# aidagroup/quad-periodic-mpc

Measured on AMD Instinct MI355X. Metric: QP solves/sec (N=10, 13-state, 12-force) at batch=65536; 1/2/4/8 GPU, higher is better.
Workload: dtype f32

## Files before the change

### quad-periodic-mpc_amd/csrc/cmpc_class1.hip

```cpp
#include <stdlib.h>

#include "cmpc_common.h"

#ifndef CMPC_W1_WAVES_60
#define CMPC_W1_WAVES_60 4
#endif
#ifndef CMPC_W1_WAVES_PER_EU
#define CMPC_W1_WAVES_PER_EU 4
#endif
#ifndef CMPC_C1_RL
#define CMPC_C1_RL 0
#endif
#ifndef CMPC_TRIP_PRIO_AT
#define CMPC_TRIP_PRIO_AT 0
#endif
#ifndef CMPC_C1_TRIP_PRIO
#define CMPC_C1_TRIP_PRIO 2
#endif
#ifndef C1_PIPE_GRP
#define C1_PIPE_GRP 4
#endif
#ifndef CMPC_C1_CHOL2
#define CMPC_C1_CHOL2 1
#endif
// ... 54 lines not shown
  static constexpr int PSZ = 4 * NG * NV - 8 * NG * (NG - 1);
  __host__ __device__ static constexpr int prow(int r) {
    return 4 * (r >> 2) * NV - 8 * (r >> 2) * ((r >> 2) - 1) + (r & 3) * (NV - 4 * (r >> 2));
  }
  __host__ __device__ static constexpr int prow0(int r) { return prow(r) - (r & ~3); }
  __host__ __device__ static constexpr int tri(int r) { return r * NV - ((r * (r + 1)) >> 1); }
  static_assert(NV * NV - ((NV * (NV + 1)) >> 1) <= 4 * NG * NV - 8 * NG * (NG - 1), "exchange fits P");
};
__device__ __forceinline__ int rcol(int j) { return (j * (j + 1)) >> 1; }
constexpr int rinv_cols(int words) {
  int q = 0;
  while ((q + 1) * (q + 2) <= words) q++;
  return q;
}

constexpr int OFF_E = 0;
constexpr int OFF_ZE = OFF_E + 16 * MAXN;
constexpr int OFF_REC = OFF_ZE + 16 * MAXN;

constexpr int C1_MAXFS = 24;

template <int NV>
struct SharedC1 {
  static_assert(NV % 4 == 0 && NV <= NL, "row width");
  static_assert(NV * (NV + 1) / 2 <= C1Geo<NV>::PSZ, "R must fit in P");
  static_assert(OFF_REC + CMPC_REC_WORDS(MAXN) <= C1Geo<NV>::PSZ, "prep scratch must fit in P");
  static_assert(3 * C1_MAXFS >= NV, "stance list");
  static_assert(NV * (NV + 1) / 2 <= C1Geo<NV>::PSZ - NL, "vbuf in P's tail");
  __device__ __forceinline__ float* vbuf() { return &P[C1Geo<NV>::PSZ - NL]; }
  static constexpr int QI = rinv_cols(C1Geo<NV>::PSZ - NL);
  static constexpr int RB = C1Geo<NV>::PSZ - NL - QI * (QI + 1) / 2;
  static_assert(QI * (QI + 1) / 2 <= RB, "R and R^-1 side by side");
  float P[C1Geo<NV>::PSZ];
  union {
    float BdtT[12][16];
    float ibuf[NL];
    struct {
      float bufA[NL], bufB[NL];
      float cs[2 * NL];
    } gi;
  } u;
  float sub[C1_MAXFS];
  int sfs[C1_MAXFS];
  int blkbase[MAXN + 2];
  unsigned char varblk[NL], varcol[NL];
  unsigned char cmask[NL];
};

__device__ __forceinline__ void lsync() {
  __builtin_amdgcn_wave_barrier();
  asm volatile("" ::: "memory");
}

__device__ __forceinline__ float fdiv(float a, float b) { return a * fast_rcp(b); }

template <int M>
__device__ __forceinline__ void pin(float (&x)[M]) {
#pragma unroll
  for (int c = 0; c < M; c++) asm volatile("" : "+v"(x[c]));
}

template <int LO, int HI, int MA>
__device__ __forceinline__ float pick_col(const float (&x)[MA], int q) {
  static_assert(0 <= LO && LO < HI && HI <= MA, "column range");
  if constexpr (HI - LO == 1) {
    float r = x[LO];
    asm volatile("" : "+v"(r));
    return r;
  } else {
    constexpr int MID = (LO + HI) / 2;
    if (q < MID) return pick_col<LO, MID>(x, q);
    return pick_col<MID, HI>(x, q);
  }
}

#ifndef CMPC_FENCE_COLS
#define CMPC_FENCE_COLS 16
#endif
#define CMPC_SWEEP_FENCE(c)                                                                  \
  do {                                                                                       \
    if (((c) & (CMPC_FENCE_COLS - 1)) == CMPC_FENCE_COLS - 4) __builtin_amdgcn_sched_barrier(0); \
  } while (0)

template <int NV>
__device__ __forceinline__ void solve_c1(const float* __restrict__ rec, const KParams& P,
                                         SharedC1<NV>& sh, float* __restrict__ fout,
                                         uint8_t* __restrict__ st_out, int32_t* __restrict__ it_out,
                                         int* __restrict__ ovf_list, int* __restrict__ ovf_count,
                                         int inst) {
  using G = C1Geo<NV>;
  const int v = threadIdx.x;
  const int N = P.N;
#ifdef CMPC_PHASE_PROF
  unsigned long long ph[16] = {0, 0, 0, 0, 0, 0, 0, 0, 0, 0, 0, 0, 0, 0, 0, 0};
  unsigned long long t_sub = 0;
  unsigned long long t_last = clock64();
#endif
  {
    const float4* src = reinterpret_cast<const float4*>(rec);
    float4* dst = reinterpret_cast<float4*>(&sh.P[OFF_REC]);
    for (int t = v; t < (P.rec_words >> 2); t += 64) dst[t] = src[t];
  }
  lsync();
  const float* srec = &sh.P[OFF_REC];
  const unsigned char* gait = reinterpret_cast<const unsigned char*>(srec + CMPC_REC_HDR + 12 * N);
  int nfs = 0;
  unsigned long long msk0 = 0ull, msk1 = 0ull;
  for (int c0 = 0; c0 < 4 * N; c0 += 64) {
    const int t = c0 + v;
    float ub = 0.f;
    bool f = false;
    if (t < 4 * N) {
      ub = (float)gait[t] * P.f_max;
      f = !(ub < 0.01f && ub > -0.01f);
    }
    const unsigned long long m = __ballot(f);
    if (c0 == 0) msk0 = m; else msk1 = m;
    const int pre = __popcll(m & ((1ull << v) - 1ull));
    if (f && nfs + pre < C1_MAXFS) {
      sh.sfs[nfs + pre] = t;
      sh.sub[nfs + pre] = ub;
    }
    nfs += __popcll(m);
  }
  const int n = 3 * nfs;
  if (n > NV) {
    if (v == 0 && ovf_list) ovf_list[atomicAdd(ovf_count, 1)] = inst;
    return;
  }
  lsync();
  {
    int kb = 0, kc = 0;
    if (v < n) {
      const int fs = sh.sfs[v / 3];
      kb = fs >> 2;
      kc = 3 * (fs & 3) + v % 3;
    }
    sh.varblk[v] = (unsigned char)kb;
    sh.varcol[v] = (unsigned char)kc;
    if (v <= N) {
      const int b0 = 4 * v, b1 = 4 * v - 64;
      const unsigned long long lo = (b0 >= 64) ? msk0 : (msk0 & ((1ull << b0) - 1ull));
      const unsigned long long hi = (b1 <= 0) ? 0ull : (msk1 & ((1ull << b1) - 1ull));
      sh.blkbase[v] = 3 * (__popcll(lo) + __popcll(hi));
    }
    for (int t = v; t < nfs; t += 64) sh.cmask[t] = 0;
  }
  Model md;
  make_model(srec, P.dt, md);
  make_bdt<64>(srec, md, v, sh.u.BdtT);
  CondGeo cg;
  make_cond_geo<true>(srec, md, cg);
  lsync();
  if (v < N) {
    float e[13];
    state_error(srec, md, v, srec + CMPC_REC_HDR + 12 * v, e);
#pragma unroll
    for (int j = 0; j < 13; j++) sh.P[OFF_E + 16 * v + j] = e[j];
  }
  lsync();
  float wts[13];
#pragma unroll
  for (int j = 0; j < 12; j++) wts[j] = P.wts[j];
  wts[12] = 0.f;
  {
    float ze[13];
#pragma unroll
    for (int j = 0; j < 13; j++) ze[j] = 0.f;
    for (int i = N - 1; i >= 0; i--) {
      float e[13];
#pragma unroll
      for (int j = 0; j < 13; j++) e[j] = sh.P[OFF_E + 16 * i + j];
      recur(md, wts, e, ze);
      float mine = 0.f;
#pragma unroll
      for (int j = 0; j < 13; j++) mine = (v == j) ? ze[j] : mine;
      if (v < 13) sh.P[OFF_ZE + 16 * i + v] = mine;
    }
  }
  lsync();
  C1_MARK(0);

  const bool real = v < n;
  float gv;
  {
    const int kv = real ? sh.varblk[v] : 0;
    const int cv = real ? sh.varcol[v] : 0;
    float b[13], u1[13], u2[13];
#pragma unroll
    for (int j = 0; j < 13; j++) b[j] = real ? sh.u.BdtT[cv][j] : 0.f;
    n1_mul(md, b, u1);
    n1_mul(md, u1, u2);
    {
      float zk[13];
#pragma unroll
      for (int j = 0; j < 13; j++) zk[j] = sh.P[OFF_ZE + 16 * kv + j];
      gv = real ? 2.f * dot13(b, zk) : 0.f;
    }
    lsync();
    const int myrow = G::tri(v);
    float z[13];
#pragma unroll
    for (int j = 0; j < 13; j++) z[j] = 0.f;
    for (int i = N - 1; i >= 0; i--) {
      const bool act = real && (i >= kv);
      const float k = (float)(i - kv);
      const float k2 = 0.5f * k * (k - 1.f);
      float gk[13];
      col_power(b, u1, u2, k, k2, gk);
#pragma unroll
      for (int j = 0; j < 13; j++) gk[j] = act ? gk[j] : 0.f;
      recur(md, wts, gk, z);
      asm volatile("" ::: "memory");
      const int wb = __builtin_amdgcn_readfirstlane(sh.blkbase[i]);
      step_entries(md, cg, sh.u.BdtT, step_mask(msk0, msk1, i), wb, z, [&](int w, float val) {
        if (w == v) val += P.alpha2;
        if (act && w >= v) sh.P[myrow + w] = val;
      });
    }
  }
  lsync();
  C1_MARK(1);

  float slot[NV + 1];
  {
    const int vv = (v < NV) ? v : 0;
    const int myrow = G::tri(vv);
    static_for<0, NV>([&](auto C) {
      constexpr int c = decltype(C)::value;
      const int addr = (c >= vv) ? myrow + c : G::tri(c) + vv;
      const float x = sh.P[addr];
      slot[c] = (real && c < n) ? x : ((c == v) ? 1.f : 0.f);
      if ((c & 7) == 7) __builtin_amdgcn_sched_barrier(0);
    });
    slot[NV] = gv;
  }
  lsync();

  int status = CMPC_OK;
  float my_inv = 1.f;
#if CMPC_C1_CHOL2
  float i0n = 1.f, betan = 0.f, i1n = 1.f, g0n = 0.f, g1n = 0.f;
  auto look = [&](auto JJ) {
    constexpr int j = decltype(JJ)::value, j1 = j + 1;
    constexpr int cj = j & ~3, cj1 = j1 & ~3;
    if constexpr (j1 < NV) {
    float d0 = rl(slot[j], j);
    const float h10 = rl(slot[j], j1);
    if (!(d0 > 0.f)) { status = CMPC_NOT_PD; d0 = 1e-30f; }
    i0n = __builtin_amdgcn_rsqf(d0);
    betan = h10 * (i0n * i0n);
    float d1 = fmaf(-h10, betan, rl(slot[j1], j1));
    if (!(d1 > 0.f)) { status = CMPC_NOT_PD; d1 = 1e-30f; }
    i1n = __builtin_amdgcn_rsqf(d1);
    g0n = rl(slot[NV], j);
    g1n = fmaf(-betan, g0n, rl(slot[NV], j1));
    const float s1 = fmaf(-slot[j], betan, slot[j1]);
#if CMPC_C1_FUSEDJ
    g0n = -g0n * i0n;
    g1n = -g1n * i1n;
    if (v >= cj && v < NV) sh.P[G::prow(j) + v - cj] = (v >= j) ? -slot[j] * i0n : 0.f;
    if (v >= cj1 && v < NV) sh.P[G::prow(j1) + v - cj1] = (v >= j1) ? -s1 * i1n : 0.f;
#else
    if (v >= cj && v < NV) sh.P[G::prow(j) + v - cj] = (v >= j) ? slot[j] : 0.f;
    if (v >= cj1 && v < NV) sh.P[G::prow(j1) + v - cj1] = (v >= j1) ? s1 : 0.f;
#endif
    lsync();
    }
  };
  if (n > 0) look(std::integral_constant<int, 0>{});
  float jc2 = 0.f, jc3 = 0.f;
  (void)jc2; (void)jc3;
  float xunc = 0.f;
  (void)xunc;
  static_for<0, NV / 2>([&](auto KB) {
    constexpr int k = 2 * decltype(KB)::value;
    constexpr int k1 = k + 1, k2 = k + 2;
    constexpr int c0 = k & ~3, c1 = k1 & ~3, c2 = k2 & ~3;
    constexpr int rk = G::prow(k), rk1 = G::prow(k1);
    if (k < n) {
      const float i0 = i0n, beta = betan, i1 = i1n, g0 = g0n, g1 = g1n;
#if CMPC_C1_FUSEDJ
      if (v == k) my_inv = i0;
      if (v == k1) my_inv = i1;
      const float s0 = slot[k];
      const float s1 = fmaf(-s0, beta, slot[k1]);
      const float a0 = (v > k) ? s0 * i0 : 0.f;
      const float a1 = (v > k1) ? s1 * i1 : 0.f;
#else
      if (v == k) { my_inv = i0; sh.u.ibuf[k] = i0; }
      if (v == k1) { my_inv = i1; sh.u.ibuf[k1] = i1; }
      const float s0 = slot[k];
      const float s1 = fmaf(-s0, beta, slot[k1]);
      const float a0 = (v > k) ? -s0 * (i0 * i0) : 0.f;
      const float a1 = (v > k1) ? -s1 * (i1 * i1) : 0.f;
#endif
      slot[NV] = fmaf(a1, g1, fmaf(a0, g0, slot[NV]));
      static_for<c2 / 4, NV / 4>([&](auto JC) {
        constexpr int c = 4 * decltype(JC)::value;
        const float4 r0 = *reinterpret_cast<const float4*>(&sh.P[rk + c - c0]);
        const float4 r1 = *reinterpret_cast<const float4*>(&sh.P[rk1 + c - c1]);
        axpy4(a0, r0, slot[c + 0], slot[c + 1], slot[c + 2], slot[c + 3]);
        axpy4(a1, r1, slot[c + 0], slot[c + 1], slot[c + 2], slot[c + 3]);
        if constexpr (k2 < NV && c == c2) {
          if (k2 < n) look(std::integral_constant<int, k2>{});
        }
        CMPC_SWEEP_FENCE(c);
      });
#if CMPC_C1_FUSEDJ == 2
      if constexpr ((k & 3) == 0) {
        f2v t0 = {(v == k) ? 1.f : 0.f, 0.f}, t1 = {(v == k1) ? 1.f : 0.f, 0.f};
        f2v t2 = {(v == k + 2) ? 1.f : 0.f, 0.f}, t3 = {(v == k + 3) ? 1.f : 0.f, 0.f};
#if CMPC_C1_JPIPE
        piped_sweep<0, k, 1>(
            [&](auto C) {
              constexpr int q = decltype(C)::value;
              return F4x4{*reinterpret_cast<const float4*>(&sh.P[G::prow(q) + k - q]),
                          *reinterpret_cast<const float4*>(&sh.P[G::prow(q + 1) + k - q]),
                          *reinterpret_cast<const float4*>(&sh.P[G::prow(q + 2) + k - q]),
                          *reinterpret_cast<const float4*>(&sh.P[G::prow(q + 3) + k - q])};
            },
            [&](auto C, F4x4 l) {
              constexpr int q = decltype(C)::value;
              const float4 la = l.a, lb = l.b, lc = l.c, ld = l.d;
#else
        static_for<0, k / 4>([&](auto QC) {
          constexpr int q = 4 * decltype(QC)::value;
          const float4 la = *reinterpret_cast<const float4*>(&sh.P[G::prow(q) + k - q]);
          const float4 lb = *reinterpret_cast<const float4*>(&sh.P[G::prow(q + 1) + k - q]);
          const float4 lc = *reinterpret_cast<const float4*>(&sh.P[G::prow(q + 2) + k - q]);
          const float4 ld = *reinterpret_cast<const float4*>(&sh.P[G::prow(q + 3) + k - q]);
#endif
          t0.x = fmaf(slot[q], la.x, t0.x); t1.x = fmaf(slot[q], la.y, t1.x);
          t2.x = fmaf(slot[q], la.z, t2.x); t3.x = fmaf(slot[q], la.w, t3.x);
          t0.y = fmaf(slot[q + 1], lb.x, t0.y); t1.y = fmaf(slot[q + 1], lb.y, t1.y);
          t2.y = fmaf(slot[q + 1], lb.z, t2.y); t3.y = fmaf(slot[q + 1], lb.w, t3.y);
          t0.x = fmaf(slot[q + 2], lc.x, t0.x); t1.x = fmaf(slot[q + 2], lc.y, t1.x);
          t2.x = fmaf(slot[q + 2], lc.z, t2.x); t3.x = fmaf(slot[q + 2], lc.w, t3.x);
          t0.y = fmaf(slot[q + 3], ld.x, t0.y); t1.y = fmaf(slot[q + 3], ld.y, t1.y);
          t2.y = fmaf(slot[q + 3], ld.z, t2.y); t3.y = fmaf(slot[q + 3], ld.w, t3.y);
#if CMPC_C1_JPIPE
            });
#else
          __builtin_amdgcn_sched_barrier(0);
        });
#endif
        const float hk = sh.P[G::prow(k) + k1 - (k & ~3)];
        const float xk = (t0.x + t0.y) * i0;
        slot[k] = xk;
        slot[k1] = fmaf(xk, hk, t1.x + t1.y) * i1;
#if CMPC_C1_XUNC
// ... 502 lines not shown
```

### quad-periodic-mpc_amd/csrc/cmpc_common.h

```cpp
#pragma once
#include <hip/hip_runtime.h>
#include <stdint.h>

#include <type_traits>

#include "cmpc_kernels.h"

namespace cmpc {
namespace {

constexpr int MAXN = CMPC_MAX_HORIZON;
constexpr float kBigF = 3.0e38f;

__device__ __forceinline__ float rl(float x, int lane) {
  return __int_as_float(__builtin_amdgcn_readlane(__float_as_int(x), lane));
}
__device__ __forceinline__ int rli(int x, int lane) { return __builtin_amdgcn_readlane(x, lane); }

constexpr int kDppQuadSwap1 = 0xB1;
constexpr int kDppQuadSwap2 = 0x4E;
constexpr int kDppRowShl = 0x100;
constexpr int kDppRowShr = 0x110;
constexpr int kDppWaveShl1 = 0x130;
constexpr int kDppWaveShr1 = 0x138;
// ... 56 lines not shown
  const int row = lane >> 4;
  return v + ((row == 0) ? r1 + (r2 + r3) : (row == 1) ? r2 + r3 : (row == 2) ? r3 : 0.f);
}
__device__ __forceinline__ float lane_prev(float old, float v) { return dppf<kDppWaveShr1>(old, v); }
__device__ __forceinline__ float lane_next(float old, float v) { return dppf<kDppWaveShl1>(old, v); }
__device__ __forceinline__ int lane_next_i(int old, int v) { return dppi<kDppWaveShl1>(old, v); }

__device__ __forceinline__ int tid_opq() {
  int x = threadIdx.x;
  asm volatile("" : "+v"(x));
  return x;
}

#ifndef CMPC_LANE_ASM
#define CMPC_LANE_ASM 1
#endif
__device__ __forceinline__ int lane_opq() {
#if CMPC_LANE_ASM
  int x;
  asm volatile("v_mbcnt_lo_u32_b32 %0, -1, 0\n\tv_mbcnt_hi_u32_b32 %0, -1, %0" : "=v"(x));
#else
  int x = (int)__builtin_amdgcn_mbcnt_hi(~0u, __builtin_amdgcn_mbcnt_lo(~0u, 0u));
  asm volatile("" : "+v"(x));
#endif
  return x;
}

template <int I, int E, class F>
__device__ __forceinline__ void static_for(F&& f) {
  if constexpr (I < E) {
    f(std::integral_constant<int, I>{});
    static_for<I + 1, E>(f);
  }
}
template <int C0, int CE, int GRP, class Ld, class F>
__device__ __forceinline__ void piped_sweep(Ld&& ld, F&& f) {
  constexpr int NCH = (CE > C0) ? (CE - C0) / 4 : 0;
  if constexpr (NCH > 0) {
    using T = decltype(ld(std::integral_constant<int, C0>{}));
    constexpr int NG = (NCH + GRP - 1) / GRP;
    T cur[GRP], nxt[GRP];
    static_for<0, GRP>([&](auto I) {
      constexpr int ch = decltype(I)::value;
      if constexpr (ch < NCH) cur[ch] = ld(std::integral_constant<int, C0 + 4 * ch>{});
    });
    static_for<0, NG>([&](auto GI) {
      constexpr int g = decltype(GI)::value;
      static_for<0, GRP>([&](auto I) {
        constexpr int ch = (g + 1) * GRP + decltype(I)::value;
        if constexpr (ch < NCH) nxt[decltype(I)::value] = ld(std::integral_constant<int, C0 + 4 * ch>{});
      });
      __builtin_amdgcn_sched_barrier(0);
      static_for<0, GRP>([&](auto I) {
        constexpr int ch = g * GRP + decltype(I)::value;
        if constexpr (ch < NCH) f(std::integral_constant<int, C0 + 4 * ch>{}, cur[decltype(I)::value]);
      });
      __builtin_amdgcn_sched_barrier(0);
      static_for<0, GRP>([&](auto I) { cur[decltype(I)::value] = nxt[decltype(I)::value]; });
    });
  }
}
struct F4x2 {
  float4 a, b;
};
struct F4x4 {
  float4 a, b, c, d;
};

__device__ __forceinline__ float vopq(float x) {
  asm volatile("" : "+v"(x));
  return x;
}
__device__ __forceinline__ float sopq(float x) {
  asm volatile("" : "+s"(x));
  return x;
}
__device__ __forceinline__ float rfl(float x) {
  return __int_as_float(__builtin_amdgcn_readfirstlane(__float_as_int(x)));
}
__device__ __forceinline__ int opaque(int x) {
  x = __builtin_amdgcn_readfirstlane(x);
  asm volatile("" : "+s"(x));
  return x;
}
__device__ __forceinline__ float fast_rcp(float x) { return __builtin_amdgcn_rcpf(x); }

typedef float f2v __attribute__((ext_vector_type(2)));
__device__ __forceinline__ void axpy4(float a, float4 r, float& x0, float& x1, float& x2, float& x3) {
  x0 = fmaf(a, r.x, x0);
  x1 = fmaf(a, r.y, x1);
  x2 = fmaf(a, r.z, x2);
  x3 = fmaf(a, r.w, x3);
}
__device__ __forceinline__ void dot4(f2v& acc, float x0, float x1, float x2, float x3, float4 r) {
  acc.x = fmaf(x0, r.x, acc.x);
  acc.x = fmaf(x1, r.y, acc.x);
  acc.x = fmaf(x2, r.z, acc.x);
  acc.x = fmaf(x3, r.w, acc.x);
}
__device__ __forceinline__ void dot4x2(f2v& acc, float x0, float x1, float x2, float x3, float4 r) {
  acc.x = fmaf(x0, r.x, acc.x);
  acc.y = fmaf(x1, r.y, acc.y);
  acc.x = fmaf(x2, r.z, acc.x);
  acc.y = fmaf(x3, r.w, acc.y);
}

__device__ __forceinline__ void wsync() {
  __builtin_amdgcn_fence(__ATOMIC_RELEASE, "workgroup");
  __builtin_amdgcn_wave_barrier();
  __builtin_amdgcn_fence(__ATOMIC_ACQUIRE, "workgroup");
}

struct Model {
  float R[9];
  float n1r[9];
  float dt, dth, xdrag;
};

__device__ __forceinline__ void n1_mul(const Model& m, const float* x, float* y) {
#pragma unroll
  for (int i = 0; i < 3; i++) y[i] = m.n1r[i * 3 + 0] * x[6] + m.n1r[i * 3 + 1] * x[7] + m.n1r[i * 3 + 2] * x[8];
  y[3] = m.dt * x[9];
  y[4] = m.dt * x[10];
  y[5] = m.dt * x[11] + (m.dth * m.xdrag) * x[9] + m.dth * x[12];
#pragma unroll
  for (int i = 6; i < 11; i++) y[i] = 0.f;
  y[11] = (m.dt * m.xdrag) * x[9] + m.dt * x[12];
  y[12] = 0.f;
}

__device__ __forceinline__ void recur(const Model& m, const float* wts, const float* e, float* z) {
  float t[13];
#pragma unroll
  for (int j = 0; j < 13; j++) t[j] = z[j];
  const float c6 = m.n1r[0] * t[0] + m.n1r[3] * t[1] + m.n1r[6] * t[2];
  const float c7 = m.n1r[1] * t[0] + m.n1r[4] * t[1] + m.n1r[7] * t[2];
  const float c8 = m.n1r[2] * t[0] + m.n1r[5] * t[1] + m.n1r[8] * t[2];
  const float c9 = m.dt * t[3] + (m.dt * m.xdrag) * t[11] + (m.dth * m.xdrag) * t[5];
  const float c10 = m.dt * t[4];
  const float c11 = m.dt * t[5];
  const float c12 = m.dt * t[11] + m.dth * t[5];
#pragma unroll
  for (int j = 0; j < 13; j++) z[j] = wts[j] * e[j] + t[j];
  z[6] += c6; z[7] += c7; z[8] += c8; z[9] += c9; z[10] += c10; z[11] += c11; z[12] += c12;
}

__device__ __forceinline__ float dot13(const float* a, const float* b) {
  float s = 0.f;
#pragma unroll
  for (int j = 0; j < 13; j++) s = fmaf(a[j], b[j], s);
  return s;
}

__device__ __forceinline__ unsigned step_mask(unsigned long long m0, unsigned long long m1, int i) {
  return (unsigned)(((i < 16) ? (m0 >> (4 * i)) : (m1 >> (4 * i - 64))) & 15ull);
}

#ifndef CMPC_COND_DOT13
#define CMPC_COND_DOT13 0
#endif

struct CondGeo {
  float Ii[9];
  float r[12];
};
struct StepProj {
  float w[3], p[3];
};

__device__ __forceinline__ void make_iinv(const Model& md, float* Ii) {
  const float Ib0 = .07f, Ib1 = 0.26f, Ib2 = 0.242f;
  float Iw[9];
#pragma unroll
  for (int i = 0; i < 3; i++)
#pragma unroll
    for (int j = 0; j < 3; j++)
      Iw[i * 3 + j] = md.R[i * 3 + 0] * Ib0 * md.R[j * 3 + 0] + md.R[i * 3 + 1] * Ib1 * md.R[j * 3 + 1] +
                      md.R[i * 3 + 2] * Ib2 * md.R[j * 3 + 2];
  const float c00 = Iw[4] * Iw[8] - Iw[5] * Iw[7];
  const float c10 = Iw[5] * Iw[6] - Iw[3] * Iw[8];
  const float c20 = Iw[3] * Iw[7] - Iw[4] * Iw[6];
  const float idet = 1.f / (Iw[0] * c00 + Iw[1] * c10 + Iw[2] * c20);
  Ii[0] = c00 * idet; Ii[1] = (Iw[2] * Iw[7] - Iw[1] * Iw[8]) * idet; Ii[2] = (Iw[1] * Iw[5] - Iw[2] * Iw[4]) * idet;
  Ii[3] = c10 * idet; Ii[4] = (Iw[0] * Iw[8] - Iw[2] * Iw[6]) * idet; Ii[5] = (Iw[2] * Iw[3] - Iw[0] * Iw[5]) * idet;
  Ii[6] = c20 * idet; Ii[7] = (Iw[1] * Iw[6] - Iw[0] * Iw[7]) * idet; Ii[8] = (Iw[0] * Iw[4] - Iw[1] * Iw[3]) * idet;
}

template <bool UNIFORM, typename RecPtr>
__device__ __forceinline__ void make_cond_geo(RecPtr rec, const Model& md, CondGeo& cg) {
  make_iinv(md, cg.Ii);
#pragma unroll
  for (int j = 0; j < 12; j++) cg.r[j] = rec[CMPC_REC_R + j];
  if constexpr (UNIFORM) {
#pragma unroll
    for (int j = 0; j < 9; j++) cg.Ii[j] = rfl(cg.Ii[j]);
#pragma unroll
    for (int j = 0; j < 12; j++) cg.r[j] = rfl(cg.r[j]);
  }
}

__device__ __forceinline__ void step_proj(const Model& md, const CondGeo& cg, const float* z, StepProj& pj) {
  const float dt2 = 2.f * md.dt, dtq = 2.f * md.dth, dtc = md.dt * md.dt * md.dt / 3.f;
  const float im = 1.f / 12.0f;
  float q[3];
#pragma unroll
  for (int i = 0; i < 3; i++)
    q[i] = fmaf(dt2, z[6 + i], dtq * fmaf(md.R[i * 3 + 2], z[2], fmaf(md.R[i * 3 + 1], z[1], md.R[i * 3] * z[0])));
#pragma unroll
  for (int j = 0; j < 3; j++)
    pj.w[j] = fmaf(cg.Ii[6 + j], q[2], fmaf(cg.Ii[3 + j], q[1], cg.Ii[j] * q[0]));
#pragma unroll
  for (int a = 0; a < 3; a++) pj.p[a] = im * fmaf(dt2, z[9 + a], dtq * z[3 + a]);
  pj.p[0] = fmaf(im * md.xdrag, fmaf(dtq, z[11], dtc * z[5]), pj.p[0]);
}

__device__ __forceinline__ void foot_entries(const StepProj& pj, float r0, float r1, float r2, float* out) {
  out[0] = fmaf(pj.w[1], r2, fmaf(-pj.w[2], r1, pj.p[0]));
  out[1] = fmaf(pj.w[2], r0, fmaf(-pj.w[0], r2, pj.p[1]));
  out[2] = fmaf(pj.w[0], r1, fmaf(-pj.w[1], r0, pj.p[2]));
}

__device__ __forceinline__ void col_power(const float* b, const float* u1, const float* u2, float k, float k2,
                                          float* e) {
#pragma unroll
  for (int j = 0; j < 5; j++) e[j] = fmaf(k, u1[j], b[j]);
  e[5] = fmaf(k2, u2[5], fmaf(k, u1[5], b[5]));
#pragma unroll
  for (int j = 6; j < 11; j++) e[j] = b[j];
  e[11] = fmaf(k, u1[11], b[11]);
  e[12] = b[12];
}

template <class St>
__device__ __forceinline__ void step_columns(const CondGeo& cg, unsigned mi, int wb, const StepProj& pj,
                                             St&& st) {
  int w = wb;
  static_for<0, 4>([&](auto F) {
    constexpr int f = decltype(F)::value;
    if (mi & (1u << f)) {
      float val[3];
      foot_entries(pj, cg.r[f], cg.r[4 + f], cg.r[8 + f], val);
      st(w, val[0]);
      st(w + 1, val[1]);
      st(w + 2, val[2]);
      w += 3;
    }
  });
}
template <class St>
__device__ __forceinline__ void step_columns_dot13(const float (*BdtT)[16], unsigned mi, int wb,
                                                   const float* z, St&& st) {
  int w = wb;
  static_for<0, 4>([&](auto F) {
    constexpr int f = decltype(F)::value;
    if (mi & (1u << f)) {
      static_for<0, 3>([&](auto A) {
        constexpr int c = 3 * f + decltype(A)::value;
        float bw[16];
#pragma unroll
        for (int q = 0; q < 4; q++) {
          const float4 b4 = *reinterpret_cast<const float4*>(&BdtT[c][4 * q]);
          bw[4 * q] = b4.x; bw[4 * q + 1] = b4.y; bw[4 * q + 2] = b4.z; bw[4 * q + 3] = b4.w;
        }
        st(w, 2.f * dot13(bw, z));
        w++;
      });
    }
  });
}
template <class St>
__device__ __forceinline__ void step_entries(const Model& md, const CondGeo& cg, const float (*BdtT)[16],
                                             unsigned mi, int wb, const float* z, St&& st) {
#if CMPC_COND_DOT13
  step_columns_dot13(BdtT, mi, wb, z, st);
#else
  StepProj pj;
  step_proj(md, cg, z, pj);
  step_columns(cg, mi, wb, pj, st);
#endif
}

__device__ __forceinline__ void make_model(const float* __restrict__ rec, float dt, Model& md) {
  const float qw = rec[CMPC_REC_Q + 0], qx = rec[CMPC_REC_Q + 1], qy = rec[CMPC_REC_Q + 2],
              qz = rec[CMPC_REC_Q + 3];
  const float tx = 2.f * qx, ty = 2.f * qy, tz = 2.f * qz;
  const float twx = tx * qw, twy = ty * qw, twz = tz * qw;
  const float txx = tx * qx, txy = ty * qx, txz = tz * qx;
  const float tyy = ty * qy, tyz = tz * qy, tzz = tz * qz;
  md.R[0] = 1.f - (tyy + tzz); md.R[1] = txy - twz;         md.R[2] = txz + twy;
  md.R[3] = txy + twz;         md.R[4] = 1.f - (txx + tzz); md.R[5] = tyz - twx;
  md.R[6] = txz - twy;         md.R[7] = tyz + twx;         md.R[8] = 1.f - (txx + tyy);
  md.dt = dt;
  md.dth = dt * dt * 0.5f;
  md.xdrag = rec[CMPC_REC_XDRAG];
#pragma unroll
  for (int i = 0; i < 3; i++)
#pragma unroll
    for (int j = 0; j < 3; j++) md.n1r[i * 3 + j] = dt * md.R[j * 3 + i];
}

template <int NT>
__device__ __forceinline__ void make_bdt(const float* __restrict__ rec, const Model& md, int tid,
                                         float (*BdtT)[16]) {
  static_assert(NT >= 12, "one thread per force column");
  if (tid < 12) {
    float Ii[9];
// ... 114 lines not shown
```

### quad-periodic-mpc_amd/csrc/cmpc_condense.hip

```cpp
#include "cmpc_common.h"

namespace cmpc {
namespace {

constexpr int NTG = 256;

struct SharedC {
  float BdtT[12][16];
  float traj[12 * MAXN];
  float E[MAXN][16];
  float ZE[MAXN][16];
};

__device__ void condense_one(const float* __restrict__ rec, const KParams& P, SharedC& sh,
                             float* __restrict__ H, float* __restrict__ g) {
  const int tid = threadIdx.x;
  const int N = P.N;
  const int n = 12 * N;
  for (int t = tid; t < 12 * N; t += NTG) sh.traj[t] = rec[CMPC_REC_HDR + t];
  Model md;
  make_model(rec, P.dt, md);
  make_bdt<NTG>(rec, md, tid, sh.BdtT);
  CondGeo cg;
  make_cond_geo<true>(rec, md, cg);
  __syncthreads();
  if (tid < N) {
    float e[13];
    state_error(rec, md, tid, &sh.traj[12 * tid], e);
#pragma unroll
    for (int j = 0; j < 13; j++) sh.E[tid][j] = e[j];
  }
  __syncthreads();
  float wts[13];
#pragma unroll
  for (int j = 0; j < 12; j++) wts[j] = P.wts[j];
  wts[12] = 0.f;
  if (tid < 64) {
    float ze[13];
#pragma unroll
    for (int j = 0; j < 13; j++) ze[j] = 0.f;
    for (int i = N - 1; i >= 0; i--) {
      float e[13];
#pragma unroll
      for (int j = 0; j < 13; j++) e[j] = sh.E[i][j];
      recur(md, wts, e, ze);
      if ((tid & 63) == 0) {
#pragma unroll
        for (int j = 0; j < 13; j++) sh.ZE[i][j] = ze[j];
      }
    }
  }
  __syncthreads();
  for (int v = tid; v < n; v += NTG) {
    const int kv = v / 12, cv = v - 12 * (v / 12);
    float b[13], u1[13], u2[13];
#pragma unroll
    for (int j = 0; j < 13; j++) b[j] = sh.BdtT[cv][j];
    n1_mul(md, b, u1);
    n1_mul(md, u1, u2);
    {
      float zk[13];
#pragma unroll
      for (int j = 0; j < 13; j++) zk[j] = sh.ZE[kv][j];
      g[v] = 2.f * dot13(b, zk);
    }
    float z[13];
#pragma unroll
    for (int j = 0; j < 13; j++) z[j] = 0.f;
    for (int i = N - 1; i >= kv; i--) {
      const float k = (float)(i - kv);
      const float k2 = 0.5f * k * (k - 1.f);
      float gk[13];
      col_power(b, u1, u2, k, k2, gk);
      recur(md, wts, gk, z);
      step_entries(md, cg, sh.BdtT, 15u, 12 * i, z, [&](int w, float val) {
        if (w == v) val += P.alpha2;
#ifdef CMPC_DIAG_PERTURB
        val *= 1.f + CMPC_DIAG_PERTURB;
#endif
        if (w >= v) {
          H[(size_t)v * n + w] = val;
          H[(size_t)w * n + v] = val;
        }
      });
    }
  }
}

__global__ __launch_bounds__(NTG) void cmpc_condense_kernel(const float* __restrict__ recs, int batch, KParams P,
                                                            float* __restrict__ Hout, float* __restrict__ gout) {
  __shared__ SharedC sh;
  const size_t n = 12 * (size_t)P.N;
  for (int inst = blockIdx.x; inst < batch; inst += gridDim.x) {
    condense_one(recs + (size_t)inst * P.rec_words, P, sh, Hout + inst * n * n, gout + inst * n);
    __syncthreads();
  }
}

}

hipError_t launch_condense(const float* d_recs, int batch, const KParams& P, float* d_H, float* d_g,
                           hipStream_t stream) {
  if (batch <= 0) return hipSuccess;
  const int grid = batch < 2048 ? batch : 2048;
  hipLaunchKernelGGL(cmpc_condense_kernel, dim3(grid), dim3(NTG), 0, stream, d_recs, batch, P, d_H, d_g);
  return hipGetLastError();
}

}
```

### quad-periodic-mpc_amd/csrc/cmpc_wide.h

```cpp
#pragma once
#include "cmpc_common.h"

#ifndef CMPC_DIAG_STOP
#define CMPC_DIAG_STOP 0
#endif
#ifndef CMPC_WIDE_WAVES_PER_EU
#define CMPC_WIDE_WAVES_PER_EU 3
#endif
#ifndef CMPC_WIDE_CHOL2
#define CMPC_WIDE_CHOL2 1
#endif
#ifndef CMPC_WIDE_J2
#define CMPC_WIDE_J2 CMPC_WIDE_CHOL2
#endif
#ifndef CMPC_WIDE_SKIP
#define CMPC_WIDE_SKIP 1
#endif
#ifndef CMPC_WIDE_VGPR_CAP
#define CMPC_WIDE_VGPR_CAP 0
#endif
#ifndef CMPC_WIDE_REFINE
#define CMPC_WIDE_REFINE 1
#endif
#ifndef CMPC_TRIP_PRIO_AT
// ... 409 lines not shown
      }
    }
    wbar();
    if (t < 6 * N) scr[S0 + 12 * (t / 6) + t - 6 * (t / 6)] = ev;
  }
  wbar();
}

template <int NV>
__device__ __forceinline__ void wide_refine(const float* __restrict__ rec_in, const KParams& P, SharedW<NV>& sh,
                                            float (&slot)[WGeo<NV>::NH], float& xv, int q, int n, int wave) {
  using G = WGeo<NV>;
  constexpr int NH = G::NH;
  constexpr int NC = (NH + 63) / 64;
  const gfloat* rec = (const gfloat*)(rec_in);
  asm volatile("" : "+s"(rec));
  double* scr = reinterpret_cast<double*>(&sh.P[G::O_RINV]);
  refine_residual<NV>(rec_in, P, sh, wave);
  float rr = 0.f;
  {
    CMPC_WIDE_IDS();
    if (r < n) {
      const int k = sh.varblk[r], c = sh.varcol[r];
      const int b = c / 3, a = c - 3 * (c / 3);
      const int a1 = (a == 2) ? 0 : a + 1, a2 = (a == 0) ? 2 : a - 1;
      const double* yk = scr + 24 + 12 * k;
      const double cr = yk[a1] * (double)rec[CMPC_REC_R + 4 * a2 + b] - yk[a2] * (double)rec[CMPC_REC_R + 4 * a1 + b];
      rr = (float)(2.0 * (cr + yk[3 + a]) + (double)sopq(P.alpha2) * (double)xv);
    }
  }
  float pa[NC], pb[NC];
#pragma unroll
  for (int m = 0; m < NC; m++) { pa[m] = 0.f; pb[m] = 0.f; }
  if (!(CMPC_DIAG_REF_SKIP & 16)) {
    const int ln = lane_opq();
    static_for<0, NH>([&](auto JC) {
      constexpr int j = decltype(JC)::value;
      float v = slot[j] * rr;
      v += dppf<kDppQuadSwap1>(0.f, v);
      v += dppf<kDppQuadSwap2>(0.f, v);
      v += dppf<kDppRowHalfMirror>(0.f, v);
      v += dppf<kDppRowMirror>(0.f, v);
      v += dppf<kDppRowBcast15, 0xa>(0.f, v);
      const float s0 = rl(v, 31), s1 = rl(v, 63);
      if (ln == (j & 63)) { pa[j >> 6] = s0; pb[j >> 6] = s1; }
      if ((j & 3) == 3) __builtin_amdgcn_sched_barrier(0);
    });
    float* ub = sh.vbuf();
    for (int w = 0; w < G::NW; w++) {
      if (wave == w) {
        const bool last = (w == G::NW - 1);
#pragma unroll
        for (int m = 0; m < NC; m++) {
          const int l = 64 * m + ln;
          if (l < NH) {
            float u0 = pa[m] + (w ? ub[l] : 0.f);
            float u1 = pb[m] + (w ? ub[G::HOFF + l] : 0.f);
            if (last) {
              u0 = (l >= q && l < n) ? u0 : 0.f;
              u1 = (NH + l >= q && NH + l < n) ? u1 : 0.f;
            }
            ub[l] = u0;
            ub[G::HOFF + l] = u1;
          }
        }
      }
      wbar();
    }
  }
  {
    CMPC_WIDE_IDS();
    f2v acc = {0.f, 0.f};
    const float* vb = &sh.vbuf()[h * G::HOFF];
#pragma unroll
    for (int j = 0; j < NH; j += 4) {
      const float4 u4 = *reinterpret_cast<const float4*>(vb + j);
      dot4(acc, slot[j + 0], slot[j + 1], slot[j + 2], slot[j + 3], u4);
      CMPC_WSWEEP_FENCE(j);
    }
    const float dx = pair_sum(acc.x + acc.y);
    if (r < n && !(CMPC_DIAG_REF_SKIP & 16)) xv -= dx;
  }
}

template <int NV, bool REFINE>
__device__ __forceinline__ void solve_w(const float* __restrict__ rec, const KParams& P,
                                        SharedW<NV>& sh, float* __restrict__ fout,
                                        uint8_t* __restrict__ st_out, int32_t* __restrict__ it_out) {
  using G = WGeo<NV>;
  constexpr int NH = G::NH;
  constexpr int RQ = G::RQ;
  constexpr int kGiFence = (NH <= 48) ? 8 : 16;
  const int t = tid_opq();
  const int lane = t & 63;
  const int wave = __builtin_amdgcn_readfirstlane(t >> 6);
  const int h = lane >> 5;
  const int r = 32 * wave + (lane & 31);
  const int N = P.N;
  {
    const float4* src = reinterpret_cast<const float4*>(rec);
    float4* dst = reinterpret_cast<float4*>(&sh.P[W_OFF_REC]);
    for (int i = t; i < (P.rec_words >> 2); i += G::NT) dst[i] = src[i];
  }
  wbar();
  const float* srec = &sh.P[W_OFF_REC];
  const unsigned char* gait = reinterpret_cast<const unsigned char*>(srec + CMPC_REC_HDR + 12 * N);
  int nfs = 0;
  unsigned long long msk0 = 0ull, msk1 = 0ull;
  for (int c0 = 0; c0 < 4 * N; c0 += 64) {
    const int s = c0 + lane;
    float ub = 0.f;
    bool f = false;
    if (s < 4 * N) {
      ub = (float)gait[s] * P.f_max;
      f = !(ub < 0.01f && ub > -0.01f);
      if (wave == 0) sh.stance[s] = f ? 1 : 0;
    }
    const unsigned long long m = __ballot(f);
    if (c0 == 0) msk0 = m; else msk1 = m;
    const int pre = __popcll(m & ((1ull << lane) - 1ull));
    if (f && wave == 0) {
      sh.sfs[nfs + pre] = s;
      sh.sub[nfs + pre] = ub;
    }
    nfs += __popcll(m);
  }
  const int n = 3 * nfs;
  if (n > NV) {
    if (t == 0) { st_out[0] = CMPC_BAD_INPUT; if (it_out) it_out[0] = 0; }
    return;
  }
  wbar();
  {
    int kb = 0, kc = 0;
    if (t < n) {
      const int fs = sh.sfs[t / 3];
      kb = fs >> 2;
      kc = 3 * (fs & 3) + t % 3;
    }
    sh.varblk[t] = (unsigned char)kb;
    sh.varcol[t] = (unsigned char)kc;
    if (t <= N) {
      const int b0 = 4 * t, b1 = 4 * t - 64;
      const unsigned long long lo = (b0 >= 64) ? msk0 : (msk0 & ((1ull << b0) - 1ull));
      const unsigned long long hi = (b1 <= 0) ? 0ull : (msk1 & ((1ull << b1) - 1ull));
      sh.blkbase[t] = 3 * (__popcll(lo) + __popcll(hi));
    }
    for (int i = t; i < 6 * nfs; i += G::NT) sh.cflag[i] = 0;
  }
  Model md;
  make_model(srec, P.dt, md);
  make_bdt<G::NT>(srec, md, t, sh.BdtT());
  wbar();
  if (t < N) {
    float e[13];
    state_error(srec, md, t, srec + CMPC_REC_HDR + 12 * t, e);
#pragma unroll
    for (int j = 0; j < 13; j++) sh.P[W_OFF_E + 16 * t + j] = e[j];
  }
  wbar();
  float wts[13];
#pragma unroll
  for (int j = 0; j < 12; j++) wts[j] = P.wts[j];
  wts[12] = 0.f;
  {
    float ze[13];
#pragma unroll
    for (int j = 0; j < 13; j++) ze[j] = 0.f;
    for (int i = N - 1; i >= 0; i--) {
      float e[13];
#pragma unroll
      for (int j = 0; j < 13; j++) e[j] = sh.P[W_OFF_E + 16 * i + j];
      recur(md, wts, e, ze);
      float mine = 0.f;
#pragma unroll
      for (int j = 0; j < 13; j++) mine = (t == j) ? ze[j] : mine;
      if (t < 13) sh.P[W_OFF_ZE + 16 * i + t] = mine;
    }
  }
  wbar();

  const bool real = r < n;
  const int rr = (r < NV) ? r : 0;
  float gv;
  {
    const int kv = real ? sh.varblk[r] : 0;
    const int cv = real ? sh.varcol[r] : 0;
    float b[13], u1[13], u2[13];
#pragma unroll
    for (int j = 0; j < 13; j++) b[j] = real ? sh.BdtT()[cv][j] : 0.f;
    n1_mul(md, b, u1);
    n1_mul(md, u1, u2);
    {
      float zk[13];
#pragma unroll
      for (int j = 0; j < 13; j++) zk[j] = sh.P[W_OFF_ZE + 16 * kv + j];
      gv = real ? 2.f * dot13(b, zk) : 0.f;
    }
    wbar();
    const int myrow = G::tri(rr);
    float z[13];
#pragma unroll
    for (int j = 0; j < 13; j++) z[j] = 0.f;
    for (int i = N - 1; i >= 0; i--) {
      const bool act = real && (i >= kv);
      const float k = (float)(i - kv);
      const float k2 = 0.5f * k * (k - 1.f);
      float gk[13];
#pragma unroll
      for (int j = 0; j < 13; j++) gk[j] = act ? fmaf(k2, u2[j], fmaf(k, u1[j], b[j])) : 0.f;
      recur(md, wts, gk, z);
      const int wb = __builtin_amdgcn_readfirstlane(sh.blkbase[i]);
      const int we = __builtin_amdgcn_readfirstlane(sh.blkbase[i + 1]);
      for (int w0 = wb; w0 < we; w0 += 2) {
        const int w = w0 + h;
        const int cw = sh.varcol[w];
        float bw[13];
#pragma unroll
        for (int j = 0; j < 13; j++) bw[j] = sh.BdtT()[cw][j];
        float val = 2.f * dot13(bw, z);
        if (w == r) val += P.alpha2;
        if (act && w < we && w >= r) sh.P[myrow + w] = val;
      }
    }
  }
  wbar();

  float slot[NH];
  float gb = gv;
  {
    const int myrow = G::tri(rr);
    static_for<0, NH>([&](auto J) {
      constexpr int j = decltype(J)::value;
      const int c = 2 * j + h;
      const int addr = (c >= rr) ? myrow + c : G::tri(c) + rr;
      const float x = sh.P[addr];
      slot[j] = (real && c < n) ? x : ((c == r) ? 1.f : 0.f);
      if ((j & 7) == 7) __builtin_amdgcn_sched_barrier(0);
    });
  }
  wbar();

  int status = CMPC_OK;
  float my_inv = 1.f;
#if CMPC_DIAG_STOP != 3
#if CMPC_WIDE_CHOL2
  static_for<0, NV / 2>([&](auto KB) {
    constexpr int k = 2 * decltype(KB)::value, k1 = k + 1;
    constexpr int kj = k >> 1;
    constexpr int j0 = G::j0(k);
    constexpr int base = G::fbase(k), base1 = G::fbase(k1);
    constexpr int st = G::seg(k);
    if (k < n) {
      CMPC_WIDE_IDS();
      const float mine = slot[kj];
      const float other = pair_other(mine, h);
      const float hk = h ? other : mine;
      const float hk1 = h ? mine : other;
      if (h == 0 && r >= 2 * j0 && r < NV) sh.P[base + (r & 1) * st + (r >> 1) - j0] = (r >= k) ? mine : 0.f;
      if (h == 1 && r >= 2 * j0 && r < NV) sh.P[base1 + (r & 1) * st + (r >> 1) - j0] = (r >= k1) ? mine : 0.f;
      if (h == 0 && (r == k || r == k1)) sh.gbuf()[r] = gb;
      wbar();
      float d0 = sh.P[base + kj - j0];
      const float h10 = sh.P[base + st + kj - j0];
      const float d1r = sh.P[base1 + st + kj - j0];
      const float g0 = sh.gbuf()[k], g1 = sh.gbuf()[k1];
      if (!(d0 > 0.f)) { status = CMPC_NOT_PD; d0 = 1e-30f; }
      const float i0 = __builtin_amdgcn_rsqf(d0);
      const float beta = h10 * (i0 * i0);
      float d1 = fmaf(-h10, beta, d1r);
      if (!(d1 > 0.f)) { status = CMPC_NOT_PD; d1 = 1e-30f; }
      const float i1 = __builtin_amdgcn_rsqf(d1);
      if (r == k) { my_inv = i0; if (h == 0) sh.ibuf()[k] = i0; }
      if (r == k1) { my_inv = i1; if (h == 0) sh.ibuf()[k1] = i1; }
      const float s1 = fmaf(-hk, beta, hk1);
      const float a1 = (r > k1 && r < NV) ? -s1 * (i1 * i1) : 0.f;
      const float a0 = (r > k && r < NV) ? fmaf(-a1, beta, -hk * (i0 * i0)) : 0.f;
      if (CMPC_WIDE_SKIP == 0 || (32 * wave + 31 > k && 32 * wave < n)) {
        const float* prow0 = &sh.P[base + h * st - j0];
        const float* prow1 = &sh.P[base1 + h * st - j0];
#pragma unroll
        for (int j = j0; j < NH; j += 4) {
          const float4 r0 = *reinterpret_cast<const float4*>(prow0 + j);
          const float4 r1 = *reinterpret_cast<const float4*>(prow1 + j);
          axpy4(a0, r0, slot[j + 0], slot[j + 1], slot[j + 2], slot[j + 3]);
          axpy4(a1, r1, slot[j + 0], slot[j + 1], slot[j + 2], slot[j + 3]);
          CMPC_WSWEEP2_FENCE(j);
        }
        gb = fmaf(a1, g1, fmaf(a0, g0, gb));
      }
      wpin(slot);
    }
  });
#else
  static_for<0, NV>([&](auto KC) {
    constexpr int k = decltype(KC)::value;
    constexpr int kj = k >> 1, kh = k & 1;
    constexpr int j0 = G::j0(k);
    constexpr int base = G::fbase(k);
    constexpr int st = G::seg(k);
    if (k < n) {
      const float mine = slot[kj];
      const float other = pair_other(mine, h);
      const float hrk = (h == kh) ? mine : other;
      if (h == kh && r >= 2 * j0 && r < NV)
        sh.P[base + (r & 1) * st + (r >> 1) - j0] = (r >= k) ? mine : 0.f;
      if (r == k && h == 0) sh.gbuf()[k] = gb;
      wbar();
      float d = sh.P[base + kh * st + kj - j0];
      if (!(d > 0.f)) { status = CMPC_NOT_PD; d = 1e-30f; }
      const float inv = __builtin_amdgcn_rsqf(d);
      if (r == k) { my_inv = inv; if (h == 0) sh.ibuf()[k] = inv; }
      const float a = (r > k && r < NV) ? -hrk * (inv * inv) : 0.f;
      const float* prow = &sh.P[base + h * st - j0];
#pragma unroll
      for (int j = j0; j < NH; j += 4) {
        const float4 r4 = *reinterpret_cast<const float4*>(prow + j);
        axpy4(a, r4, slot[j + 0], slot[j + 1], slot[j + 2], slot[j + 3]);
        CMPC_WSWEEP_FENCE(j);
      }
      gb = fmaf(a, sh.gbuf()[k], gb);
      wpin(slot);
    }
  });
#endif
#endif
  float yv;
  {
    CMPC_WIDE_IDS();
    yv = (r < n) ? gb * my_inv : 0.f;
    if (h == 0 && r < NV) sh.ybuf(r & 1)[r >> 1] = yv;
  }
  wbar();

#if CMPC_DIAG_STOP != 1 && CMPC_DIAG_STOP != 3
  {
    const int to = 64 * wave + lane_opq();
    const int lr = ((to & 63) >> 5) - 32 * (to >> 6) - (to & 31);
    static_for<0, NH>([&](auto J) {
      constexpr int j = decltype(J)::value;
      slot[j] = (lr == -2 * j) ? 1.f : 0.f;
    });
  }
#if CMPC_WIDE_J2
  static_for<0, NV / 2>([&](auto KB) {
    constexpr int k = 2 * decltype(KB)::value, k1 = k + 1;
    constexpr int kj = k >> 1;
    constexpr int j0 = G::j0(k);
    constexpr int base = G::fbase(k), base1 = G::fbase(k1);
    constexpr int st = G::seg(k);
    if (k < n && (CMPC_WIDE_SKIP == 0 || k1 >= 32 * wave)) {
      wlsync();
      const int h = (lane_opq() >> 5) & 1;
      const float i0 = sh.ibuf()[k], i1 = sh.ibuf()[k1];
      const float h10 = sh.P[base + st + kj - j0];
      const float beta = h10 * (i0 * i0);
      const float mine = slot[kj];
      const float other = pair_other(mine, h);
      const float x0 = (h ? other : mine) * i0;
      const float x1 = fmaf(-h10 * i0, x0, h ? mine : other) * i1;
      const float a1 = -x1 * i1;
      const float a0 = fmaf(-a1, beta, -x0 * i0);
      const float* prow0 = &sh.P[base + h * st - j0];
// ... 591 lines not shown
```

Measured before the change: 50.08 million.

## Replace backward costate recurrence for gradient with prefix-sum moment formulation

The serial backward recurrence over the horizon that built the costate vectors ZE by applying the full 13x13 model recurrence at every step is replaced. Weighted errors are now accumulated into zeroth, first and second order running sums, one lane per state component. Each variable's gradient is then reconstructed from those moments and its b/u1/u2 power-series vectors. This removes a serial chain of dense recurrence steps per problem, at the cost of relying on the dynamics' nilpotent structure (only components 5 and 11 feeding higher moments) and changed floating-point summation order.

Measured after the change: 51.12 million, median of 6. 2.1% higher.

```diff
diff --git a/quad-periodic-mpc_amd/csrc/cmpc_class1.hip b/quad-periodic-mpc_amd/csrc/cmpc_class1.hip
--- a/quad-periodic-mpc_amd/csrc/cmpc_class1.hip
+++ b/quad-periodic-mpc_amd/csrc/cmpc_class1.hip
@@ -230,32 +230,18 @@
   CondGeo cg;
   make_cond_geo<true>(srec, md, cg);
   lsync();
+  float wts[13];
+#pragma unroll
+  for (int j = 0; j < 12; j++) wts[j] = P.wts[j];
+  wts[12] = 0.f;
   if (v < N) {
     float e[13];
     state_error(srec, md, v, srec + CMPC_REC_HDR + 12 * v, e);
 #pragma unroll
-    for (int j = 0; j < 13; j++) sh.P[OFF_E + 16 * v + j] = e[j];
-  }
-  lsync();
-  float wts[13];
-#pragma unroll
-  for (int j = 0; j < 12; j++) wts[j] = P.wts[j];
-  wts[12] = 0.f;
-  {
-    float ze[13];
-#pragma unroll
-    for (int j = 0; j < 13; j++) ze[j] = 0.f;
-    for (int i = N - 1; i >= 0; i--) {
-      float e[13];
-#pragma unroll
-      for (int j = 0; j < 13; j++) e[j] = sh.P[OFF_E + 16 * i + j];
-      recur(md, wts, e, ze);
-      float mine = 0.f;
-#pragma unroll
-      for (int j = 0; j < 13; j++) mine = (v == j) ? ze[j] : mine;
-      if (v < 13) sh.P[OFF_ZE + 16 * i + v] = mine;
-    }
-  }
+    for (int j = 0; j < 13; j++) sh.P[OFF_E + 16 * v + j] = wts[j] * e[j];
+  }
+  lsync();
+  moment_recur(&sh.P[OFF_E], &sh.P[OFF_ZE], N, v);
   lsync();
   C1_MARK(0);
 
@@ -269,12 +255,8 @@
     for (int j = 0; j < 13; j++) b[j] = real ? sh.u.BdtT[cv][j] : 0.f;
     n1_mul(md, b, u1);
     n1_mul(md, u1, u2);
-    {
-      float zk[13];
-#pragma unroll
-      for (int j = 0; j < 13; j++) zk[j] = sh.P[OFF_ZE + 16 * kv + j];
-      gv = real ? 2.f * dot13(b, zk) : 0.f;
-    }
+    gv = grad_from_moments(b, u1, u2, &sh.P[OFF_E + 16 * kv], &sh.P[OFF_ZE + 16 * kv]);
+    gv = real ? gv : 0.f;
     lsync();
     const int myrow = G::tri(v);
     float z[13];
diff --git a/quad-periodic-mpc_amd/csrc/cmpc_common.h b/quad-periodic-mpc_amd/csrc/cmpc_common.h
--- a/quad-periodic-mpc_amd/csrc/cmpc_common.h
+++ b/quad-periodic-mpc_amd/csrc/cmpc_common.h
@@ -232,6 +232,36 @@
   return s;
 }
 
+constexpr int kMomM2 = 13;
+
+__device__ __forceinline__ void moment_recur(float* E, float* M, int N, int lane) {
+  if (lane < 13) {
+    float m0 = 0.f, m1 = 0.f, m2 = 0.f;
+    float we = E[16 * (N - 1) + lane];
+    for (int k = N - 1; k >= 0; k--) {
+      const float nx = (k > 0) ? E[16 * (k - 1) + lane] : 0.f;
+      m2 += m1;
+      m1 += m0;
+      m0 += we;
+      E[16 * k + lane] = m0;
+      M[16 * k + lane] = m1;
+      if (lane == 5) M[16 * k + kMomM2] = m2;
+      we = nx;
+    }
+  }
+}
+
+__device__ __forceinline__ float grad_from_moments(const float* b, const float* u1, const float* u2,
+                                                   const float* E0, const float* Mk) {
+  float s = u2[5] * Mk[kMomM2];
+  s = fmaf(u1[11], Mk[11], s);
+#pragma unroll
+  for (int j = 5; j >= 0; j--) s = fmaf(u1[j], Mk[j], s);
+#pragma unroll
+  for (int j = 0; j < 13; j++) s = fmaf(b[j], E0[j], s);
+  return 2.f * s;
+}
+
 __device__ __forceinline__ unsigned step_mask(unsigned long long m0, unsigned long long m1, int i) {
   return (unsigned)(((i < 16) ? (m0 >> (4 * i)) : (m1 >> (4 * i - 64))) & 15ull);
 }
diff --git a/quad-periodic-mpc_amd/csrc/cmpc_condense.hip b/quad-periodic-mpc_amd/csrc/cmpc_condense.hip
--- a/quad-periodic-mpc_amd/csrc/cmpc_condense.hip
+++ b/quad-periodic-mpc_amd/csrc/cmpc_condense.hip
@@ -24,32 +24,18 @@
   CondGeo cg;
   make_cond_geo<true>(rec, md, cg);
   __syncthreads();
+  float wts[13];
+#pragma unroll
+  for (int j = 0; j < 12; j++) wts[j] = P.wts[j];
+  wts[12] = 0.f;
   if (tid < N) {
     float e[13];
     state_error(rec, md, tid, &sh.traj[12 * tid], e);
 #pragma unroll
-    for (int j = 0; j < 13; j++) sh.E[tid][j] = e[j];
+    for (int j = 0; j < 13; j++) sh.E[tid][j] = wts[j] * e[j];
   }
   __syncthreads();
-  float wts[13];
-#pragma unroll
-  for (int j = 0; j < 12; j++) wts[j] = P.wts[j];
-  wts[12] = 0.f;
-  if (tid < 64) {
-    float ze[13];
-#pragma unroll
-    for (int j = 0; j < 13; j++) ze[j] = 0.f;
-    for (int i = N - 1; i >= 0; i--) {
-      float e[13];
-#pragma unroll
-      for (int j = 0; j < 13; j++) e[j] = sh.E[i][j];
-      recur(md, wts, e, ze);
-      if ((tid & 63) == 0) {
-#pragma unroll
-        for (int j = 0; j < 13; j++) sh.ZE[i][j] = ze[j];
-      }
-    }
-  }
+  moment_recur(&sh.E[0][0], &sh.ZE[0][0], N, tid);
   __syncthreads();
   for (int v = tid; v < n; v += NTG) {
     const int kv = v / 12, cv = v - 12 * (v / 12);
@@ -58,12 +44,7 @@
     for (int j = 0; j < 13; j++) b[j] = sh.BdtT[cv][j];
     n1_mul(md, b, u1);
     n1_mul(md, u1, u2);
-    {
-      float zk[13];
-#pragma unroll
-      for (int j = 0; j < 13; j++) zk[j] = sh.ZE[kv][j];
-      g[v] = 2.f * dot13(b, zk);
-    }
+    g[v] = grad_from_moments(b, u1, u2, sh.E[kv], sh.ZE[kv]);
     float z[13];
 #pragma unroll
     for (int j = 0; j < 13; j++) z[j] = 0.f;
diff --git a/quad-periodic-mpc_amd/csrc/cmpc_wide.h b/quad-periodic-mpc_amd/csrc/cmpc_wide.h
--- a/quad-periodic-mpc_amd/csrc/cmpc_wide.h
+++ b/quad-periodic-mpc_amd/csrc/cmpc_wide.h
@@ -585,32 +585,18 @@
   make_model(srec, P.dt, md);
   make_bdt<G::NT>(srec, md, t, sh.BdtT());
   wbar();
+  float wts[13];
+#pragma unroll
+  for (int j = 0; j < 12; j++) wts[j] = P.wts[j];
+  wts[12] = 0.f;
   if (t < N) {
     float e[13];
     state_error(srec, md, t, srec + CMPC_REC_HDR + 12 * t, e);
 #pragma unroll
-    for (int j = 0; j < 13; j++) sh.P[W_OFF_E + 16 * t + j] = e[j];
+    for (int j = 0; j < 13; j++) sh.P[W_OFF_E + 16 * t + j] = wts[j] * e[j];
   }
   wbar();
-  float wts[13];
-#pragma unroll
-  for (int j = 0; j < 12; j++) wts[j] = P.wts[j];
-  wts[12] = 0.f;
-  {
-    float ze[13];
-#pragma unroll
-    for (int j = 0; j < 13; j++) ze[j] = 0.f;
-    for (int i = N - 1; i >= 0; i--) {
-      float e[13];
-#pragma unroll
-      for (int j = 0; j < 13; j++) e[j] = sh.P[W_OFF_E + 16 * i + j];
-      recur(md, wts, e, ze);
-      float mine = 0.f;
-#pragma unroll
-      for (int j = 0; j < 13; j++) mine = (t == j) ? ze[j] : mine;
-      if (t < 13) sh.P[W_OFF_ZE + 16 * i + t] = mine;
-    }
-  }
+  moment_recur(&sh.P[W_OFF_E], &sh.P[W_OFF_ZE], N, tid_opq());
   wbar();
 
   const bool real = r < n;
@@ -624,12 +610,8 @@
     for (int j = 0; j < 13; j++) b[j] = real ? sh.BdtT()[cv][j] : 0.f;
     n1_mul(md, b, u1);
     n1_mul(md, u1, u2);
-    {
-      float zk[13];
-#pragma unroll
-      for (int j = 0; j < 13; j++) zk[j] = sh.P[W_OFF_ZE + 16 * kv + j];
-      gv = real ? 2.f * dot13(b, zk) : 0.f;
-    }
+    gv = grad_from_moments(b, u1, u2, &sh.P[W_OFF_E + 16 * kv], &sh.P[W_OFF_ZE + 16 * kv]);
+    gv = real ? gv : 0.f;
     wbar();
     const int myrow = G::tri(rr);
     float z[13];
@@ -640,8 +622,9 @@
       const float k = (float)(i - kv);
       const float k2 = 0.5f * k * (k - 1.f);
       float gk[13];
-#pragma unroll
-      for (int j = 0; j < 13; j++) gk[j] = act ? fmaf(k2, u2[j], fmaf(k, u1[j], b[j])) : 0.f;
+      col_power(b, u1, u2, k, k2, gk);
+#pragma unroll
+      for (int j = 0; j < 13; j++) gk[j] = act ? gk[j] : 0.f;
       recur(md, wts, gk, z);
       const int wb = __builtin_amdgcn_readfirstlane(sh.blkbase[i]);
       const int we = __builtin_amdgcn_readfirstlane(sh.blkbase[i + 1]);
```
